# rasmusab/bayes.js

Measured on AMD Instinct MI355X. Metric: posterior draws/sec (= param-updates/sec), higher is better.
Workload: dtype f64

## Files before the change

bayes.js_amd/amwg_ctypes.py:

```python
import bisect
import ctypes as C
import os

import numpy as np

HERE = os.path.dirname(os.path.abspath(__file__))
LIB_PATH = os.environ.get("AMWG_LIB") or os.path.join(HERE, "csrc", "libamwg.so")
MODEL_ID = {"normal": 1, "beta_bern": 2, "hier_normal": 3, "pois_glm": 4}


class ParamDesc(C.Structure):
    _fields_ = [("type", C.c_int32), ("len", C.c_int32), ("top", C.c_int32), ("multidim", C.c_int32),
                ("lower", C.c_double), ("upper", C.c_double)]


class CompOpt(C.Structure):
    _fields_ = [("prop_log_scale", C.c_double), ("max_adaptation", C.c_double), ("initial_adaptation", C.c_double),
                ("target_accept_rate", C.c_double), ("batch_size", C.c_double), ("is_adapting", C.c_int32)]


class ModelDesc(C.Structure):
    _fields_ = [("model", C.c_int32), ("n_obs", C.c_int32), ("x", C.POINTER(C.c_double)), ("y", C.POINTER(C.c_double)),
                ("g", C.POINTER(C.c_int32)), ("G", C.c_int32), ("K", C.c_int32), ("hyper", C.c_double * 8)]

# ... 2 lines not shown


class Options(C.Structure):
    _fields_ = [("chains", C.c_int64), ("seed", C.c_uint64), ("chain_offset", C.c_uint64), ("device", C.c_int32),
                ("lanes_per_chain", C.c_int32), ("block_threads", C.c_int32), ("steps_per_launch", C.c_int32),
                ("exact_division", C.c_int32), ("group_local", C.c_int32), ("full_evaluation", C.c_int32), ("test_bound_shift", C.c_int32), ("sufficient_statistics", C.c_int32)]


class UserModel(C.Structure):
    _fields_ = [("source", C.c_char_p), ("n_arrays", C.c_int32), ("arrays", C.POINTER(C.POINTER(C.c_double))),
                ("array_len", C.POINTER(C.c_int64)), ("array_type", C.POINTER(C.c_int32)), ("n_derived", C.c_int32), ("lds_bytes", C.c_int32), ("lds_bytes_one_lane", C.c_int32),
                ("parallel", C.c_int32), ("max_threads", C.c_int32), ("work_per_eval", C.c_double), ("work_one_lane", C.c_double),
                ("rows_n_obs", C.c_int32), ("rows_groups", C.c_int32), ("rows_sweep", C.c_int32)]


EXPORTS = ["amwg_last_sample_dataset_histogram", "amwg_set_histogram", "amwg_histogram_info", "amwg_sample_summarize","amwg_sample_summarize_async", "amwg_summary_info", "amwg_create_user_datasets", "amwg_compile_user_datasets", "amwg_create_datasets", "amwg_create_datasets_ragged", "amwg_num_datasets", "amwg_dataset_n_obs", "amwg_last_sample_dataset_moments", "amwg_last_sample_dataset_diagnostics", "amwg_last_sample_dataset_quantiles", "amwg_kernel_name", "amwg_summation_order", "amwg_group_gather_draws", "amwg_group_comm_info", "amwg_comm_unique_id", "amwg_comm_create", "amwg_comm_info", "amwg_comm_gather_draws", "amwg_comm_moments", "amwg_comm_destroy", "amwg_code_cache_stats", "amwg_tuning", "amwg_group_moments", "amwg_group_diagnostics", "amwg_group_quantiles", "amwg_last_sample_quantiles", "amwg_fp64_peak", "amwg_set_state", "amwg_last_sample_diagnostics", "amwg_create_user", "amwg_compile_user", "amwg_num_recorded", "amwg_create", "amwg_burn", "amwg_burn_async", "amwg_sample", "amwg_sample_async", "amwg_fetch_draws", "amwg_fetch_draws_slices", "amwg_sample_device", "amwg_set_adapting", "amwg_get_state", "amwg_info", "amwg_chain_diag", "amwg_last_sample_moments", "amwg_sync", "amwg_num_components", "amwg_num_chains", "amwg_launch_info", "amwg_destroy", "amwg_last_error", "amwg_version", "amwg_exp", "amwg_log", "amwg_uniform"]
SELFTEST_EXPORTS = ["amwg_histogram_check", "amwg_summaries_check","amwg_fold_check","amwg_dataset_quantiles_check", "amwg_prefault_selftest", "amwg_math1", "amwg_math2", "amwg_hypot3", "amwg_log1p", "amwg_expm1", "amwg_two_valued_sum_check", "amwg_pow", "amwg_ld_host", "amwg_ld_device", "amwg_device_eval"]

_lib = None


def lib():
    global _lib
    if _lib is None:
        if not os.path.exists(LIB_PATH):
            raise RuntimeError("libamwg.so is missing: run `python -c 'import __graft_entry__ as g; g.build()'`")
        L = C.CDLL(LIB_PATH)
        vp, i32, i64, u64, dbl = C.c_void_p, C.c_int32, C.c_int64, C.c_uint64, C.c_double
        pd, pi32, pi64, pu64 = C.POINTER(dbl), C.POINTER(i32), C.POINTER(i64), C.POINTER(u64)
        L.amwg_create.argtypes = [C.POINTER(ModelDesc), C.POINTER(ParamDesc), i32, pd, C.POINTER(CompOpt),
                                  C.POINTER(Options), C.POINTER(vp)]
# ... 18 lines not shown
        L.amwg_last_sample_dataset_histogram.argtypes = [vp, pd, i32, pu64]
        L.amwg_set_histogram.argtypes = [vp, pd, i32]
        L.amwg_histogram_info.argtypes = [vp, pi32, C.POINTER(C.c_size_t)]
        L.amwg_set_adapting.argtypes = [vp, i32]
        L.amwg_get_state.argtypes = [vp, pd, C.c_size_t]
        L.amwg_info.argtypes = [vp, pd, pi32, pi32, pi32, pi64, pi64]
        L.amwg_chain_diag.argtypes = [vp, pu64, pd, pi32]
        L.amwg_last_sample_moments.argtypes = [vp, pd, pd]
        L.amwg_sync.argtypes = [vp]
        L.amwg_num_components.argtypes = [vp]
        L.amwg_num_chains.argtypes = [vp]
        L.amwg_num_chains.restype = i64
        L.amwg_launch_info.argtypes = [vp, pi32, pi32, pi32, pi32, pi32, pd]
        L.amwg_kernel_name.argtypes = [vp]
        L.amwg_summation_order.argtypes = [vp]
        L.amwg_kernel_name.restype = C.c_char_p
        L.amwg_destroy.argtypes = [vp]
        L.amwg_last_error.restype = C.c_char_p
        L.amwg_version.restype = C.c_char_p
        L.amwg_exp.restype = dbl
        L.amwg_exp.argtypes = [dbl]
        L.amwg_log.restype = dbl
        L.amwg_log.argtypes = [dbl]
        L.amwg_uniform.restype = dbl
        L.amwg_uniform.argtypes = [u64, u64, u64]
        L.amwg_compile_user.argtypes = [C.c_char_p, i32, i32, C.c_char_p, C.POINTER(C.c_size_t)]
        L.amwg_code_cache_stats.argtypes = [pi64, pi64, C.c_char_p, C.c_size_t]
        L.amwg_create_user.argtypes = [C.POINTER(UserModel), C.POINTER(ParamDesc), i32, pd, C.POINTER(CompOpt),
                                       C.POINTER(Options), C.POINTER(vp)]
        L.amwg_create_user_datasets.argtypes = [C.POINTER(UserModel), i32, C.POINTER(ParamDesc), i32, pd, C.POINTER(CompOpt), C.POINTER(Options), C.POINTER(vp)]
# ... 328 lines not shown
        return out

    def tuning(self):
        L = lib()
        L.amwg_tuning.argtypes = [C.c_void_p, C.POINTER(C.c_int32), C.POINTER(C.c_double), C.c_int32]
        lanes, ms = (C.c_int32 * 16)(), (C.c_double * 16)()
        n = L.amwg_tuning(self.h, lanes, ms, 16)
        return [(lanes[i], ms[i]) for i in range(min(n, 16))]

    def launch_info(self):
        v = [C.c_int32() for _ in range(5)]
        ms = C.c_double()
        _check(lib().amwg_launch_info(self.h, *[C.byref(x) for x in v], C.byref(ms)))
        return {"lanes_per_chain": v[0].value, "block_threads": v[1].value, "grid_blocks": v[2].value,
                "lds_bytes": v[3].value, "n_launches": v[4].value, "kernel_ms": ms.value, "kernel": (lib().amwg_kernel_name(self.h) or b"").decode(),
                "summation_order": lib().amwg_summation_order(self.h), "datasets": lib().amwg_num_datasets(self.h)}


def _edges_per_value(edges, PR):
    e = np.asarray(edges, dtype=np.float64)
    if e.ndim == 1:
        e = np.broadcast_to(e, (PR, e.size))
    if e.ndim != 2 or e.shape[0] != PR or e.shape[1] < 1:
        raise AmwgError("edges must be [bins + 1] or [%d recorded values][bins + 1], got shape %s" % (PR, e.shape))
    return np.ascontiguousarray(e)


def histogram_check(draws, D, edges, window_rows=0, counts=None, device=0):
    dr = np.ascontiguousarray(draws, dtype=np.float64)
    rows, PR, Cn = dr.shape
    e = _edges_per_value(edges, PR)
# ... 169 lines not shown
```

bayes.js_amd/csrc/amwg_diag.hip:

```cpp
#include <cmath>
#include <cstdarg>
#include <cstdio>

#include "amwg_build_id.h"
#include "amwg_fold.h"
#include "amwg_host.h"
#include "amwg_math.h"
#include "amwg_philox.h"

using namespace amwg;

namespace {
__global__ void chain_halves_kernel(const double *draws, int64_t rows, int PR, int64_t C, double *out) {
  const int64_t c = (int64_t)blockIdx.x * blockDim.x + threadIdx.x;
  const int p = blockIdx.y;
  if (c >= C) return;
  const int64_t half = rows / 2;
  for (int h = 0; h < 2; ++h) {
    const int64_t r0 = h * half, r1 = r0 + half;
    double m = 0, m2 = 0;
    for (int64_t r = r0; r < r1; ++r) welford_add(draws[(r * PR + p) * C + c], r - r0 + 1, m, m2);
    out[((size_t)(h * 2 + 0) * PR + p) * C + c] = m;
    out[((size_t)(h * 2 + 1) * PR + p) * C + c] = half > 1 ? m2 / (double)(half - 1) : 0.0;
  }
// ... 332 lines not shown
int amwg_num_components(const amwg_sampler *s) { return s ? s->P : 0; }
int amwg_num_recorded(const amwg_sampler *s) { return s ? s->P + s->D : 0; }
int64_t amwg_num_chains(const amwg_sampler *s) { return s ? s->C : 0; }

int amwg_launch_info(const amwg_sampler *s, int32_t *lanes, int32_t *block, int32_t *grid, int32_t *lds, int32_t *n_launches, double *kernel_ms) {
  if (!s) return amwg_fail(AMWG_EINVAL, "amwg_launch_info: null sampler");
  if (lanes) *lanes = s->plan.lanes;
  if (block) *block = s->plan.block;
  if (grid) *grid = s->plan.grid;
  if (lds) *lds = s->plan.lds;
  if (n_launches) *n_launches = s->n_launches;
  if (kernel_ms) *kernel_ms = s->kernel_ms;
  return AMWG_OK;
}

int amwg_summation_order(const amwg_sampler *s) {
  if (!s) return amwg_fail(AMWG_EINVAL, "amwg_summation_order: null sampler");
  return info(s->plan.variant).certified ? 1 : s->plan.lanes;
}

const char *amwg_kernel_name(const amwg_sampler *s) {
  if (!s) { (void)amwg_fail(AMWG_EINVAL, "amwg_kernel_name: null sampler"); return ""; }
  amwg_sampler *m = const_cast<amwg_sampler *>(s);
  if (m->kernel_name.empty()) {
    const LaunchPlan &p = s->plan;
    const int cls = p.block <= 256 ? 256 : (p.block <= 512 ? 512 : 1024);
    const std::string variant_name = std::string(info(p.variant).name) + (s->n_datasets > 1 ? "_ds" : "");
    const char *name = variant_name.c_str();
    static const char *const fam[] = {"NormalModel", "BetaBernModel", "HierNormalModel", "PoisGlmModel"};
    char buf[96];
// ... 37 lines not shown
```

bayes.js_amd/csrc/amwg_kernel.h:

```cpp
#pragma once
#if !defined(__HIPCC_RTC__)
#include <hip/hip_runtime.h>
#endif

#include "amwg_div.h"
#include "amwg_ld.h"
#include "amwg_philox.h"
#include "amwg_types.h"

namespace amwg {

struct LdsLayout {
  uint32_t data, state, pls, cnt, tot, cc, adapt, pl, idx, perm, total, stride, logpls, bc, xw;
};
__host__ __device__ inline LdsLayout lds_layout(size_t data_bytes, int P, int CPB, int max_top, int n_named, bool multi = false) {
  LdsLayout L;
  uint32_t o = 0;
  L.stride = (uint32_t)P | 1u;
  L.data = o;  o += (uint32_t)((data_bytes + 15) & ~(size_t)15);
  L.state = o; o += L.stride * CPB * 8;
  L.pls = o;   o += L.stride * CPB * 8;
  L.cnt = o;   o += L.stride * CPB * 8;
  L.tot = o;   o += (L.stride * CPB * 4 + 15) & ~15u;
  L.cc = o;    o += (uint32_t)P * sizeof(CompConst);
  L.adapt = o; o += ((uint32_t)P + 7) & ~7u;
  L.pl = o;    o += (uint32_t)n_named * 20u;
  o = (o + 15) & ~15u;
  L.idx = o;   o += (max_top > 1) ? (((uint32_t)max_top * CPB * (max_top > kByteTop ? 2u : 1u) + 15) & ~15u) : 0;
  L.perm = o;  o += (n_named > kPackedNamed) ? (((uint32_t)n_named * CPB * 2u + 15) & ~15u) : 0;
  L.logpls = o; o += multi ? L.stride * CPB * 8 : 0;
  L.bc = o;     o += multi ? ((L.stride * CPB * 4 + 15) & ~15u) : 0;
  L.xw = o;     o += multi ? 2u * 16u * 8u : 0;
  L.total = (o + 15) & ~15u;
  return L;
}

template <class Model, bool FAST, int G, int U = Model::kUnroll>
__device__ __forceinline__ double pass_over_data(const typename Model::Pass &ps, int n_obs, int sub, double acc) {
  const int n_full = n_obs / G, rem = n_obs % G;
  int k = 0;
  for (; k + U <= n_full; k += U) {
    double t[U];
#pragma unroll
    for (int u = 0; u < U; ++u) t[u] = Model::template term<FAST>(ps, (k + u) * G + sub);
#pragma unroll
    for (int u = 0; u < U; ++u) acc += t[u];
  }
// ... 228 lines not shown

__device__ inline __attribute__((noinline)) int certified_test_wide(double dA, double eta, double u) {
  const double lo = dA - eta, hi = dA + eta;
  if (hi < -746.0) return -1;
  if (lo >= 0.0) return 1;
  if (!(eta < 0x1p+9) || !(u > 0x1p-60)) return 0;
  if (exp_v8(lo) * (1.0 - 0x1p-50) > u) return 1;
  if (exp_v8(hi) * (1.0 + 0x1p-50) < u) return -1;
  return 0;
}
__device__ __forceinline__ int certified_test(double dA, double eta, double ex, double u) {
  if (eta < 0x1p-7) return (ex * (1.0 - eta) > u && (u > 0.0 || dA > -700.0)) ? 1 : (ex * (1.0 + eta) < u ? -1 : 0);
  return certified_test_wide(dA, eta, u);
}

template <class Rng>
__device__ __forceinline__ double rnorm_js(Rng &rng, double mean, double sd) {
  constexpr int GU = Rng::kLanesPerChain;
  double u, v, q;
  bool again;
  do {
    u = rng.next();
    v = 1.7156 * (rng.next() - 0.5);
    const double x = u - 0.449871;
    const double y = __builtin_fabs(v) + 0.386595;
    q = x * x + y * (0.19600 * y - 0.25472 * x);
    again = false;
    if (chain_true<GU>(q > 0.27597)) again = chain_true<GU>(q > 0.27846) || chain_true<GU>(v * v > -4 * log_v8_cold(u) * u * u);
  } while (again);
  return (v / u) * sd + mean;
}

// ... 10 lines not shown
};
__device__ __forceinline__ uint32_t perm_get(uint64_t perm, int i) { return (uint32_t)(perm >> (4 * i)) & 0xFu; }
__device__ __forceinline__ uint64_t perm_swap(uint64_t perm, int i, int j) {
  const uint64_t d = ((perm >> (4 * i)) ^ (perm >> (4 * j))) & 0xFull;
  return perm ^ (d << (4 * i)) ^ (d << (4 * j));
}

__device__ __forceinline__ double js_max2(double a, double b) {
  if (a != a || b != b) return __builtin_nan("");
  if (a == b) return (a == 0 && __builtin_signbit(a)) ? b : a;
  return a > b ? a : b;
}

template <class M, int G, bool GL, bool SW = false> struct RngOf { using type = CoopStream<G>; };
template <class M, int G> struct RngOf<M, G, true, false> { using type = typename M::Stream; };
template <class M, int G> struct RngOf<M, G, false, true> { using type = typename M::SweepStream; };
template <class M, class = void> struct DynamicLdsOf { static constexpr bool value = false; };
template <class M> struct DynamicLdsOf<M, void_of<decltype(M::kDynamicLds)>> { static constexpr bool value = M::kDynamicLds; };
template <class M, bool GL> struct DataBytesOf {
  static __device__ __forceinline__ size_t get(const DataRef &d, int lanes, int threads) {
    if constexpr (DynamicLdsOf<M>::value) return M::lds_bytes_of(d, lanes, threads);
    else return M::lds_bytes(d.n_obs, d.G, lanes);
  }
};
template <class M> struct DataBytesOf<M, true> { static __device__ __forceinline__ size_t get(const DataRef &d, int, int threads) { return M::gl_lds_bytes(d.pad, threads / 64); } };

#if defined(__HIP_DEVICE_COMPILE__)
typedef const StepArgs __attribute__((address_space(4))) *cold_args_ptr;
__device__ __forceinline__ cold_args_ptr cold_args() {
  cold_args_ptr p = (cold_args_ptr)__builtin_amdgcn_kernarg_segment_ptr();
// ... 104 lines not shown
template <class M, class = void> struct MirrorCheckOf { static constexpr bool value = false; };
template <class M> struct MirrorCheckOf<M, void_of<decltype(M::kMirrorCheck)>> { static constexpr bool value = M::kMirrorCheck; };

template <class Model, int G, int BT = 256, bool GL = false, bool SW = false, bool CT = false>
__device__ __forceinline__ void step_body(const StepArgs &a, unsigned char *smem) {
  constexpr int kPassU = SW ? (CertNeedsRows<Model>::value ? 2 : 4) : (BT >= 1024 ? 4 : 8);
  const int tid = threadIdx.x, nt = blockDim.x;
  constexpr bool kMulti = G > 64;
  if (!kMulti && a.cpb > 0 && nt != 64) { device_error(a, kErrReplicasNeedOneWave); return; }
  if (a.n_steps > 65535) { device_error(a, kErrLaunchTooLong); return; }
  const int CPB = kMulti ? G / 64 : ((a.cpb > 0 && a.cpb < nt / G) ? a.cpb : nt / G);
  const int c_raw = kMulti ? tid / 64 : tid / G;
  const int c_in = c_raw < CPB ? c_raw : CPB - 1, sub = tid % G;
  const int P = a.pl.P;
  const int n_named = a.pl.n_params;
  const LdsLayout L = lds_layout(DataBytesOf<Model, GL>::get(a.d, G, nt), P, CPB, a.pl.max_top, n_named, kMulti);

  const unsigned char *data_lds = smem + L.data;
  double *Sblk = reinterpret_cast<double *>(smem + L.state);
  CompConst *cc = reinterpret_cast<CompConst *>(smem + L.cc);
  uint8_t *adapt = smem + L.adapt;
  int32_t *pl_base = reinterpret_cast<int32_t *>(smem + L.pl), *pl_len = pl_base + n_named, *pl_top = pl_len + n_named, *pl_multidim = pl_top + n_named, *pl_inner = pl_multidim + n_named;
  const bool wide_idx = a.pl.max_top > kByteTop, wide_perm = n_named > kPackedNamed;
  const IndexColumn idx{smem + L.idx + (wide_idx ? 2 * c_in : c_in), CPB, wide_idx};
  const IndexColumn pcol{smem + L.perm + 2 * c_in, CPB, true};
  double *SDme = reinterpret_cast<double *>(smem + L.pls) + (size_t)c_in * L.stride;
  int2 *CNTme = reinterpret_cast<int2 *>(smem + L.cnt) + (size_t)c_in * L.stride;
  uint32_t *TOTme = reinterpret_cast<uint32_t *>(smem + L.tot) + (size_t)c_in * L.stride;
  double *LOGPLSme = reinterpret_cast<double *>(smem + L.logpls) + (size_t)c_in * L.stride;
  int32_t *BCme = reinterpret_cast<int32_t *>(smem + L.bc) + (size_t)c_in * L.stride;
  CrossWave xw{reinterpret_cast<double *>(smem + L.xw), 0};
// ... 11 lines not shown
  const bool counter = sub == 0 && c_raw < CPB;
  const int64_t C = a.C;

  double *Sme = Sblk + (size_t)c_in * L.stride;
  for (int p = 0; p < P; ++p) {
    Sme[p] = a.ch.state[p * C + cl];
    SDme[p] = exp_v8(a.ch.prop_log_scale[p * C + cl]);
    CNTme[p] = make_int2(a.ch.acceptance_count[p * C + cl], a.ch.iterations_since_adaption[p * C + cl]);
    TOTme[p] = 0u;
    if constexpr (kMulti) { LOGPLSme[p] = a.ch.prop_log_scale[p * C + cl]; BCme[p] = a.ch.batch_count[p * C + cl]; }
  }
  const StateView S{Sme};
  uint64_t perm = wide_perm ? 0ull : a.ch.perm[cl];
  if (wide_perm)
    for (int k = 0; k < n_named; ++k) pcol.set(k, (int)a.ch.perm16[(int64_t)k * C + cl]);
  typename RngOf<Model, G, GL, SW>::type rng;
  if constexpr (GL) rng.init(a.seed, a.chain_offset + (uint64_t)cl, a.ch.rng_n[cl], tid, reinterpret_cast<double *>(smem + L.data + Model::gl_lds_bytes(a.d.pad, 0)) + (size_t)(tid >> 6) * 256);
  else if constexpr (SW) rng.init(a.seed, a.chain_offset + (uint64_t)cl, a.ch.rng_n[cl], tid, reinterpret_cast<double *>(smem + L.data + Model::window_offset(a.d, nt / 64)) + (size_t)(tid >> 6) * 256);
  else rng.init(a.seed, a.chain_offset + (uint64_t)cl, a.ch.rng_n[cl], tid);
  double lp_curr = a.ch.lp_curr[cl];
  __syncthreads();
  constexpr bool kCert = CT && CertifiedAt<Model, G>::value && !GL && (SW == CertNeedsRows<Model>::value);
  static_assert(kCert == CT, "a certified kernel is instantiated for a model that has no certified value at this lane count");
  constexpr bool kRefOrder = kCert && G > 1 && RefOrderOf<Model>::value;
  auto expression = [&]() -> double {
    if constexpr (kRefOrder) return Model::template reference_order<G>(cache, S, a.mc, a.d, data_lds, sub);
    else if constexpr (!GL) return log_post<Model, G, kPassU>(S, a, data_lds, sub, xw, cache);
    else return 0.0;
  };
  if constexpr (!GL) { if (a.init_lp) lp_curr = expression(); }
  double lpA = lp_curr, epsA = 0.0;
  bool lp_exact = true;
  if constexpr (kCert) { if (!a.init_lp) { epsA = a.ch.lp_eps[cl]; lp_exact = epsA == 0.0; } }
// ... 595 lines not shown
        if (counter) (void)__hip_atomic_fetch_add(&TOTme[comp], 1u + ((now != old) ? 0x10000u : 0u), __ATOMIC_RELAXED, __HIP_MEMORY_SCOPE_WORKGROUP);
        if (slot + 1 < P_stepped) nx = prefetch(next_comp());
        continue;
      }
      AMWG_PHASE(14);
      const double cur = me.cur;
      const bool in_sweep = kSweep && sw_left > 0;
      double prop;
      if (in_sweep) prop = lane_value(sw_prop, comp - sb);
      else {
        prop = rnorm_js(rng, cur, me.sd);
        if (chain_true<G>(k_type == kTypeInt)) prop = js_round(prop);
      }
      const bool inb = chain_true<G>(!(prop < k_lower || prop > k_upper));
      double u_accept = 0.0;
      if (inb) { set_state(comp, prop); u_accept = in_sweep ? lane_value(sw_u, comp - sb) : rng.next(); }
      if (in_sweep) --sw_left;
      AMWG_PHASE(8);
      if (slot + 1 < P_stepped) nx = prefetch(next_comp());
      AMWG_PHASE(9);
      bool accepted = false;
      bool certified = false;
      [[maybe_unused]] double aud_E_prop = 0.0;
      if constexpr (kCert) {
        if (__ballot(inb) != 0ull) {
          wave_priority(0);
          const typename Model::Approx r = Model::template log_post_approx<G, BT>(cache, S, a.mc, a.d, data_lds, sub);
          wave_priority(kStepperPriority);
          AMWG_PHASE(10);
          if (inb) {
// ... 130 lines not shown
```

bayes.js_amd/csrc/amwg_plan.hip:

```cpp
#include <algorithm>
#include <cmath>
#include <cstdlib>

#include "amwg_host.h"
#include "amwg_kernel.h"
#include "amwg_models.h"

using namespace amwg;

const FamilyRow *family_of(int model) {
  static const FamilyRow rows[4] = {amwg_family_row<0>(), amwg_family_row<1>(), amwg_family_row<2>(), amwg_family_row<3>()};
  return model >= AMWG_MODEL_NORMAL && model <= AMWG_MODEL_POIS_GLM ? &rows[model - 1] : nullptr;
}

int gl_layout(const double *y, const int32_t *g, int N, int Gn, GlLayoutHost *out) {
  if (Gn < 1 || Gn > 64) return amwg_fail(AMWG_EINVAL, "group_local: 1 to 64 groups (a chain runs on one wavefront, a lane serves one group), got %d", Gn);
  std::vector<int> n(Gn, 0), L(Gn, 1), first(Gn, 0);
  for (int i = 0; i < N; ++i) {
    if (g[i] < 0 || g[i] >= Gn) return amwg_fail(AMWG_EINVAL, "group_local: g[%d] = %d outside 0..%d", i, g[i], Gn - 1);
    n[g[i]]++;
  }
  int total = Gn;
  for (;;) {
    int best = 0;
// ... 80 lines not shown
  return p.variant == Variant::HierSweep || p.variant == Variant::HierSweepCert || (s->user && p.pad > 0);
}

static uint32_t lds_of_size(const amwg_sampler *s, const LaunchPlan &p, int cpb, int n_obs) {
  const int G = p.lanes, bt = p.block;
  size_t data = 0;
  switch (p.variant) {
    case Variant::GroupLocal: data = HierGlModel::gl_lds_bytes(p.pad, bt / 64); break;
    case Variant::HierSweep: case Variant::HierSweepCert: data = HierNormalModel::rows_lds_bytes(p.pad, bt / 64, s->d.G); break;
    case Variant::Step: case Variant::StepCert:
      data = (s->model == AMWG_MODEL_NORMAL && G == 1) ? (p.pad ? NormalModel::one_lane_tile_bytes(n_obs) : 0) : family_of(s->model)->lds_bytes(n_obs, s->d.G, G);
      break;
    default:
      data = p.pad ? HierNormalModel::rows_lds_bytes(p.pad, bt / 64, s->user_rows_groups) : (size_t)(G == 1 ? s->user_lds_one_lane : s->user_lds);
  }
  return G > 64 ? lds_layout(data, s->P, G / 64, s->pl.max_top, s->n_params, true).total : lds_layout(data, s->P, cpb ? cpb : bt / G, s->pl.max_top, s->n_params).total;
}

static uint32_t lds_of(const amwg_sampler *s, const LaunchPlan &p, int cpb = 0) {
  if (s->n_datasets <= 1) return lds_of_size(s, p, cpb, s->d.n_obs);
  uint32_t most = 0;
  int last = -1;
  for (int n : s->ds_n_obs) {
    if (n == last) continue;
    most = std::max(most, lds_of_size(s, p, cpb, n));
    last = n;
  }
  return most;
}

static int priced_n_obs(const amwg_sampler *s) {
// ... 43 lines not shown
  return bytes / (64 * sizeof(double));
}
static int size_wave_scratch(amwg_sampler *s) {
  const char *env = getenv("AMWG_WAVE_SCRATCH");
  if ((env && env[0] == '0') || s->plan.lanes != 1) return AMWG_OK;
  const size_t lines = (size_t)s->plan.grid * (size_t)(s->plan.block / 64);
  if (s->d.wave_scratch && lines <= wave_scratch_lines(s)) return AMWG_OK;
  double *p = nullptr;
  TRYB(dev_alloc(s, &p, lines * 64));
  if (s->d.wave_scratch) {
    for (auto it = s->dev_allocs.begin(); it != s->dev_allocs.end(); ++it)
      if (*it == s->d.wave_scratch) { (void)hipFree(*it); s->dev_allocs.erase(it); break; }
  }
  s->d.wave_scratch = p;
  return AMWG_OK;
}

int choose_geometry(const amwg_sampler *s, int lanes, int n_cus, size_t max_lds, LaunchPlan *out) {
  const amwg_options &o = s->opt;
  const int max_bt = s->user ? s->user_max_threads : family_of(s->model)->max_threads;
  const int64_t cpd = chains_per_dataset(s);
  bool lds_short = false;
  auto fits = [&](int bt, int G) {
    if (bt > max_bt || bt % G != 0) return false;
    if (cpd && cpd % chains_per_workgroup(G, bt) != 0) return false;
    const LaunchPlan p = variant_for(s, G, bt, max_lds);
    if (cpd && lds_of(s, p) > max_lds) lds_short = true;
    if (lds_of(s, p) > max_lds || (bt > 512 && row_layout(s, variant_for(s, G, 512, max_lds)))) return false;
    return !(G == 1 && info(p.variant).certified && !o.block_threads && bt > (p.variant == Variant::UserStepCert ? 256 : 512));
  };
// ... 42 lines not shown
  }
  if (lanes == 0 && best.lanes > 1 && cost1 > 0 && cost1 <= 1.12 * best_cost) best = one;
  if (!best.lanes && cpd && lds_short) {
    int d_max = 0;
    for (int d = 1; d < s->n_datasets; ++d) if (s->ds_n_obs[d] > s->ds_n_obs[d_max]) d_max = d;
    return amwg_fail(AMWG_EINVAL, "no launch geometry fits dataset %d, the largest (n_obs = %d): every workgroup is given the LDS of the largest dataset, and with lanes %d (0 = any), block %d (0 = any) "
                     "that is more than %zu bytes", d_max, s->ds_n_obs[d_max], lanes, o.block_threads, max_lds);
  }
  if (!best.lanes && cpd)
    return amwg_fail(AMWG_EINVAL, "no launch geometry serves whole datasets: the chains of a workgroup (block_threads / lanes_per_chain, or 1 for a chain on several wavefronts) must divide "
                     "cpd = %lld chains per dataset; asked for lanes %d (0 = any), block %d (0 = any), %zu bytes of LDS", (long long)cpd, lanes, o.block_threads, max_lds);
  if (!best.lanes) return amwg_fail(AMWG_EINVAL, "no launch geometry fits: the model needs more than %zu bytes of LDS", max_lds);
  const int CPB = best.lanes > 64 ? 1 : (best.cpb ? best.cpb : best.block / best.lanes);
  best.grid = (int)((s->C + CPB - 1) / CPB);
  best.lds = (int)lds_of(s, best, best.cpb);
  *out = best;
  return AMWG_OK;
}

int adopt_plan(amwg_sampler *s, const LaunchPlan &p) {
  s->plan = p;
  s->d.pad = p.pad;
  if (s->user) {
    if (s->n_datasets > 1) {
      const int cpw = chains_per_workgroup(p.lanes, p.block);
      const int64_t cpd = chains_per_dataset(s);
      if (p.cpb || p.pad || (p.variant != Variant::UserStep && p.variant != Variant::UserStepCert) || cpd % cpw != 0)
        return amwg_fail(AMWG_EINVAL, "internal: a plan of %d lanes in workgroups of %d (cpb %d, pad %d) for a closure on datasets of %lld chains", p.lanes, p.block, p.cpb, p.pad, (long long)cpd);
      s->ds_blocks_per_dataset = (int)(cpd / cpw);
    }
// ... 91 lines not shown
```

bayes.js_amd/csrc/amwg_rtc.hip:

```cpp
#include <hip/hiprtc.h>
#include <fcntl.h>
#include <sys/stat.h>
#include <unistd.h>

#include <cstdio>
#include <cstdlib>
#include <cstring>
#include <map>
#include <mutex>

#include "amwg_host.h"

extern "C" {
extern const char amwg_hdr_stdint[], amwg_hdr_types[], amwg_hdr_math[], amwg_hdr_div[], amwg_hdr_ld[], amwg_hdr_philox[],
    amwg_hdr_kernel[], amwg_hdr_user[], amwg_hdr_twoval[], amwg_hdr_kval[], amwg_hdr_trig[], amwg_hdr_pass[], amwg_hdr_rows[], amwg_hdr_window[], amwg_hdr_gtail[],
    amwg_hdr_user_kernels[], amwg_hdr_user_dataset[];
}

static std::string user_program(const char *source, int lanes, int block) {
  return "#include \"amwg_kernel.h\"\n#include \"amwg_user.h\"\n#define AMWG_USER_LANES " + std::to_string(lanes) + "\n#define AMWG_USER_BLOCK " + std::to_string(block) + "\n" +
         source + "\n#include \"amwg_user_kernels.h\"\n";
}

namespace {
struct CacheKey { uint64_t h1, h2, h3; uint64_t len; };
CacheKey hash_key(const std::vector<std::string> &parts) {
  CacheKey k{0xcbf29ce484222325ull, 0x84222325cbf29ce4ull, 0x9e3779b97f4a7c15ull, 0};
  for (const std::string &p : parts) {
    for (unsigned char c : p) {
// ... 54 lines not shown
  if (!f) { close(fd); (void)remove(tmp.c_str()); return; }
  const uint64_t hdr[4] = {k.h2, k.h3, k.len, payload_sum(code)}, n = code.size();
  const bool ok = fwrite(kCacheMagic, 1, 8, f) == 8 && fwrite(hdr, 8, 4, f) == 4 && fwrite(&n, 8, 1, f) == 1 && fwrite(code.data(), 1, code.size(), f) == code.size();
  if (fclose(f) != 0 || !ok || rename(tmp.c_str(), file.c_str()) != 0) (void)remove(tmp.c_str());
}
std::atomic<int> g_cache_hits{0}, g_cache_misses{0};
}

static void dump_code_object(const std::vector<char> &code) {
  if (const char *dump = getenv("AMWG_DUMP_CODE_OBJECT")) {
    if (FILE *f = fopen(dump, "wb")) { fwrite(code.data(), 1, code.size(), f); fclose(f); }
  }
}

static int compile_user(const char *source, int lanes, int block, const char *arch, std::vector<char> *code, bool datasets, bool use_cache = true) {
  static const char *names[] = {"amwg_stdint.h", "amwg_types.h", "amwg_math.h", "amwg_div.h", "amwg_ld.h", "amwg_philox.h", "amwg_kernel.h", "amwg_user.h",
                                "amwg_twoval.h", "amwg_kval.h", "amwg_trig.h", "amwg_pass.h", "amwg_rows.h", "amwg_window.h", "amwg_gtail.h", "amwg_user_kernels.h", "amwg_user_dataset.h"};
  const char *texts[] = {amwg_hdr_stdint, amwg_hdr_types, amwg_hdr_math, amwg_hdr_div, amwg_hdr_ld, amwg_hdr_philox, amwg_hdr_kernel, amwg_hdr_user,
                         amwg_hdr_twoval, amwg_hdr_kval, amwg_hdr_trig, amwg_hdr_pass, amwg_hdr_rows, amwg_hdr_window, amwg_hdr_gtail, amwg_hdr_user_kernels, amwg_hdr_user_dataset};
  constexpr int kHeaders = (int)(sizeof(texts) / sizeof(texts[0]));
  const std::string prog_src = user_program(source, lanes, block);
#if defined(AMWG_AUDIT)
  const char *const kOpts[] = {"-O3", "-std=c++17", "-ffp-contract=off", "-fno-fast-math", "-Wno-unused-value", "-DAMWG_AUDIT=1"};
#elif defined(AMWG_X_PHASES)
  const char *const kOpts[] = {"-O3", "-std=c++17", "-ffp-contract=off", "-fno-fast-math", "-Wno-unused-value", "-DAMWG_X_PHASES=1"};
#else
  const char *const kOpts[] = {"-O3", "-std=c++17", "-ffp-contract=off", "-fno-fast-math", "-Wno-unused-value", "-falign-loops=64"};
#endif
  static const char *const kDatasetsOpt = "-DAMWG_USER_DATASETS=1";
  std::string dir = cache_dir(), file;
  CacheKey key{};
  if (!dir.empty()) {
    int rt_major = 0, rt_minor = 0;
// ... 109 lines not shown
```

bayes.js_amd/csrc/amwg_rtc_headers.c:

```c
#define AMWG_TEXT(sym, file)                                                        \
  __asm__(".section .rodata\n.global " #sym "\n.type " #sym ", @object\n" #sym ":\n" \
          ".incbin \"" file "\"\n.byte 0\n.size " #sym ", .-" #sym "\n.text\n")
AMWG_TEXT(amwg_hdr_stdint, "amwg_stdint.h");
AMWG_TEXT(amwg_hdr_types, "amwg_types.h");
AMWG_TEXT(amwg_hdr_math, "amwg_math.h");
AMWG_TEXT(amwg_hdr_div, "amwg_div.h");
AMWG_TEXT(amwg_hdr_ld, "amwg_ld.h");
AMWG_TEXT(amwg_hdr_philox, "amwg_philox.h");
AMWG_TEXT(amwg_hdr_kernel, "amwg_kernel.h");
AMWG_TEXT(amwg_hdr_user, "amwg_user.h");
AMWG_TEXT(amwg_hdr_twoval, "amwg_twoval.h");
AMWG_TEXT(amwg_hdr_kval, "amwg_kval.h");
AMWG_TEXT(amwg_hdr_trig, "amwg_trig.h");
AMWG_TEXT(amwg_hdr_pass, "amwg_pass.h");
AMWG_TEXT(amwg_hdr_rows, "amwg_rows.h");
AMWG_TEXT(amwg_hdr_window, "amwg_window.h");
AMWG_TEXT(amwg_hdr_gtail, "amwg_gtail.h");
AMWG_TEXT(amwg_hdr_user_kernels, "amwg_user_kernels.h");
AMWG_TEXT(amwg_hdr_user_dataset, "amwg_user_dataset.h");
```

bayes.js_amd/csrc/amwg_run.hip:

```cpp
#include <dlfcn.h>
#include <sys/mman.h>

#include <cmath>
#include <cstddef>
#include <cstdlib>
#include <mutex>
#include <unordered_map>

#include "../../include/amwg_selftest.h"
#include "amwg_fold.h"
#include "amwg_histogram.h"
#include "amwg_host.h"
#include "amwg_kernel.h"
#include "amwg_dataset.h"
#include "amwg_user_dataset.h"

using namespace amwg;

int use_device(int device) {
  int ndev = 0;
  hipError_t e = hipGetDeviceCount(&ndev);
  if (e != hipSuccess || ndev < 1) return amwg_fail(AMWG_EHIP, "no HIP device available (%s)", hipGetErrorString(e));
  HIP_TRY(hipSetDevice(device));
  return AMWG_OK;
// ... 32 lines not shown
  const LaunchPlan &p = s->plan;
  if (p.cpb > 0 && p.block != 64) return amwg_fail(AMWG_EINVAL, "internal: %d chains per workgroup of %d threads (replicated chains need one-wavefront workgroups)", p.cpb, p.block);
  if (p.lanes == 1 && s->d.wave_scratch && wave_scratch_lines(s) < (size_t)p.grid * (size_t)(p.block / 64))
    return amwg_fail(AMWG_EINVAL, "internal: a wave scratch of %zu lines for %d workgroups of %d threads (one line per wavefront)", wave_scratch_lines(s), p.grid, p.block);
  if (chunk > 65535) return amwg_fail(AMWG_EINVAL, "internal: launches of %lld steps (at most 65535)", (long long)chunk);
  StepArgs a{};
  a.C = s->C;
  a.seed = s->opt.seed;
  a.chain_offset = s->opt.chain_offset;
  a.thin = (int32_t)thin;
  a.draws = d_draws;
  a.cc = s->d_cc;
  a.is_adapting = s->d_adapt;
  a.pl = s->pl;
  a.cpb = p.cpb;
  a.sweep_update_by_update = s->opt.full_evaluation == 2 ? 1 : 0;
  a.certified = info(p.variant).certified ? 1 : 0;
  a.bound_scale = std::ldexp(1.0, s->opt.test_bound_shift);
  a.audit_adversarial = 0;
#if defined(AMWG_AUDIT)
  { const char *e = getenv("AMWG_AUDIT_ADVERSARIAL"); a.audit_adversarial = (e && e[0] == '1') ? 1 : 0; }
#endif
  a.mc = s->mc;
  a.d = s->d;
  if (p.lanes != 1) a.d.wave_scratch = nullptr;
  a.ch = s->ch;
  DatasetArgs ds{};
  if (s->n_datasets > 1 && !s->user) {
    if (!s->ds_kernel || s->ds_blocks_per_dataset < 1 || (int64_t)s->ds_blocks_per_dataset * s->n_datasets != p.grid)
      return amwg_fail(AMWG_EINVAL, "internal: %d workgroups for %d datasets of %d workgroups each", p.grid, s->n_datasets, s->ds_blocks_per_dataset);
// ... 387 lines not shown
```

bayes.js_amd/csrc/amwg_sampler.h:

```cpp
#pragma once
#include <hip/hip_runtime.h>

#include <cstdint>
#include <string>
#include <utility>
#include <vector>

#include "../../include/amwg.h"
#include "amwg_types.h"

typedef void (*step_kernel_t)(const amwg::StepArgs);
namespace amwg { struct DatasetArgs; struct DatasetConsts; }
typedef void (*dataset_kernel_t)(const amwg::StepArgs, const amwg::DatasetArgs);

enum class Variant : uint8_t {
  Step, StepCert, HierSweep, HierSweepCert, GroupLocal,
  UserStep, UserStepCert, UserSweep, UserSweepCert
};
struct LaunchPlan {
  int lanes = 0, block = 0, grid = 0, lds = 0, cpb = 0;
  Variant variant = Variant::Step;
  int pad = 0;
};

struct amwg_sampler {
  int device = 0;
  hipStream_t stream = nullptr;
  hipEvent_t ev0 = nullptr, ev1 = nullptr;
  int model = 0, P = 0, n_params = 0;
  int64_t C = 0;
  amwg_options opt{};
  amwg::ParamLayout pl{};
  amwg::ModelConsts mc{};
  amwg::DataRef d{};
  amwg::ChainArrays ch{};
  std::vector<void *> dev_allocs;
  amwg::CompConst *d_cc = nullptr;
// ... 45 lines not shown
```

bayes.js_amd/csrc/amwg_types.h:

```cpp
#pragma once
#include "amwg_stdint.h"

namespace amwg {

constexpr int kPackedNamed = 16;
constexpr int kByteTop = 256;
constexpr int kMaxIndex = 65535;
constexpr int kInlineUserArrays = 16;
constexpr int kTypeReal = 0, kTypeInt = 1, kTypeBinary = 2, kTypeFixed = 3;

struct StateView {
  const double *base;
#if defined(__HIPCC__)
  __host__ __device__ __forceinline__
#else
  inline
#endif
  double operator()(int p) const { return base[p]; }
};

struct CompConst {
  double lower, upper, max_adaptation, initial_adaptation, target_accept_rate;
  double batch_size;
  int32_t type;
// ... 54 lines not shown
  int64_t C;
  uint64_t seed, chain_offset;
  int32_t n_steps, thin;
  int64_t step0;
  double *draws;
  int64_t row0;
  const CompConst *cc;
  const uint8_t *is_adapting;
  int32_t init_lp;
  int32_t finalize_lp;
  int32_t certified;
  double bound_scale;
  int32_t audit_adversarial;
  int32_t sweep_update_by_update;
  int32_t cpb;
  ParamLayout pl;
  ModelConsts mc;
  DataRef d;
  ChainArrays ch;
};

}
```

include/amwg.h:

```cpp
#ifndef AMWG_H
#define AMWG_H

#include <stddef.h>
#include <stdint.h>

#ifdef __cplusplus
extern "C" {
#endif

#define AMWG_OK 0
#define AMWG_EINVAL (-1)
#define AMWG_EHIP (-2)
#define AMWG_ESIZE (-3)

enum {
  AMWG_MODEL_NORMAL = 1,
  AMWG_MODEL_BETA_BERN = 2,
  AMWG_MODEL_HIER_NORMAL = 3,
  AMWG_MODEL_POIS_GLM = 4
};

enum { AMWG_REAL = 0, AMWG_INT = 1, AMWG_BINARY = 2, AMWG_FIXED = 3 };

typedef struct {
// ... 135 lines not shown
int amwg_comm_info(amwg_comm *c, int32_t *n_ranks, int32_t *rank, int32_t *device);
int amwg_comm_gather_draws(amwg_sampler *s, amwg_comm *c, int32_t root, double *dst_device, size_t capacity_bytes, int64_t *counts);
int amwg_comm_moments(amwg_sampler *s, amwg_comm *c, double *mean, double *sd);
int amwg_comm_destroy(amwg_comm *c);

int amwg_tuning(const amwg_sampler *s, int32_t *lanes, double *ms, int32_t cap);

int amwg_sync(amwg_sampler *s);
int amwg_num_components(const amwg_sampler *s);
int amwg_num_recorded(const amwg_sampler *s);
int64_t amwg_num_chains(const amwg_sampler *s);
int amwg_launch_info(const amwg_sampler *s, int32_t *lanes_per_chain, int32_t *block_threads, int32_t *grid_blocks,
                     int32_t *lds_bytes, int32_t *n_launches, double *kernel_ms);
const char *amwg_kernel_name(const amwg_sampler *s);
int amwg_summation_order(const amwg_sampler *s);
int amwg_destroy(amwg_sampler *s);
const char *amwg_last_error(void);
const char *amwg_version(void);

double amwg_exp(double x);
double amwg_log(double x);
double amwg_uniform(uint64_t seed, uint64_t chain, uint64_t index);
int amwg_fp64_peak(int32_t device, double *lane_ops_per_s);

#ifdef __cplusplus
}
#endif
#endif
```

Measured before the change: 1.483 billion.

## Buffer Philox uniforms in an LDS ring with wave-wide refills for one-lane chains

For one-lane-per-chain stepping kernels, uniforms now come from a per-thread ring buffer in LDS. The wave refills it cooperatively, generating Philox blocks only while some lane is short, and the normal sampler's rejection loop runs wave-synchronously with predicated draws. The aim is to cut divergence from lanes calling Philox at different times and to amortize each four-word Philox block across two uniforms. In exchange it adds LDS use, ballot loops and extra bookkeeping. The ring is only granted when occupancy is not reduced, and it can be disabled with AMWG_RING=0.

```diff
diff --git a/bayes.js_amd/amwg_ctypes.py b/bayes.js_amd/amwg_ctypes.py
--- a/bayes.js_amd/amwg_ctypes.py
+++ b/bayes.js_amd/amwg_ctypes.py
@@ -40,7 +40,7 @@
                 ("rows_n_obs", C.c_int32), ("rows_groups", C.c_int32), ("rows_sweep", C.c_int32)]
 
 
-EXPORTS = ["amwg_last_sample_dataset_histogram", "amwg_set_histogram", "amwg_histogram_info", "amwg_sample_summarize","amwg_sample_summarize_async", "amwg_summary_info", "amwg_create_user_datasets", "amwg_compile_user_datasets", "amwg_create_datasets", "amwg_create_datasets_ragged", "amwg_num_datasets", "amwg_dataset_n_obs", "amwg_last_sample_dataset_moments", "amwg_last_sample_dataset_diagnostics", "amwg_last_sample_dataset_quantiles", "amwg_kernel_name", "amwg_summation_order", "amwg_group_gather_draws", "amwg_group_comm_info", "amwg_comm_unique_id", "amwg_comm_create", "amwg_comm_info", "amwg_comm_gather_draws", "amwg_comm_moments", "amwg_comm_destroy", "amwg_code_cache_stats", "amwg_tuning", "amwg_group_moments", "amwg_group_diagnostics", "amwg_group_quantiles", "amwg_last_sample_quantiles", "amwg_fp64_peak", "amwg_set_state", "amwg_last_sample_diagnostics", "amwg_create_user", "amwg_compile_user", "amwg_num_recorded", "amwg_create", "amwg_burn", "amwg_burn_async", "amwg_sample", "amwg_sample_async", "amwg_fetch_draws", "amwg_fetch_draws_slices", "amwg_sample_device", "amwg_set_adapting", "amwg_get_state", "amwg_info", "amwg_chain_diag", "amwg_last_sample_moments", "amwg_sync", "amwg_num_components", "amwg_num_chains", "amwg_launch_info", "amwg_destroy", "amwg_last_error", "amwg_version", "amwg_exp", "amwg_log", "amwg_uniform"]
+EXPORTS = ["amwg_ring_uniforms", "amwg_last_sample_dataset_histogram", "amwg_set_histogram", "amwg_histogram_info", "amwg_sample_summarize","amwg_sample_summarize_async", "amwg_summary_info", "amwg_create_user_datasets", "amwg_compile_user_datasets", "amwg_create_datasets", "amwg_create_datasets_ragged", "amwg_num_datasets", "amwg_dataset_n_obs", "amwg_last_sample_dataset_moments", "amwg_last_sample_dataset_diagnostics", "amwg_last_sample_dataset_quantiles", "amwg_kernel_name", "amwg_summation_order", "amwg_group_gather_draws", "amwg_group_comm_info", "amwg_comm_unique_id", "amwg_comm_create", "amwg_comm_info", "amwg_comm_gather_draws", "amwg_comm_moments", "amwg_comm_destroy", "amwg_code_cache_stats", "amwg_tuning", "amwg_group_moments", "amwg_group_diagnostics", "amwg_group_quantiles", "amwg_last_sample_quantiles", "amwg_fp64_peak", "amwg_set_state", "amwg_last_sample_diagnostics", "amwg_create_user", "amwg_compile_user", "amwg_num_recorded", "amwg_create", "amwg_burn", "amwg_burn_async", "amwg_sample", "amwg_sample_async", "amwg_fetch_draws", "amwg_fetch_draws_slices", "amwg_sample_device", "amwg_set_adapting", "amwg_get_state", "amwg_info", "amwg_chain_diag", "amwg_last_sample_moments", "amwg_sync", "amwg_num_components", "amwg_num_chains", "amwg_launch_info", "amwg_destroy", "amwg_last_error", "amwg_version", "amwg_exp", "amwg_log", "amwg_uniform"]
 SELFTEST_EXPORTS = ["amwg_histogram_check", "amwg_summaries_check","amwg_fold_check","amwg_dataset_quantiles_check", "amwg_prefault_selftest", "amwg_math1", "amwg_math2", "amwg_hypot3", "amwg_log1p", "amwg_expm1", "amwg_two_valued_sum_check", "amwg_pow", "amwg_ld_host", "amwg_ld_device", "amwg_device_eval"]
 
 _lib = None
@@ -89,6 +89,7 @@
         L.amwg_launch_info.argtypes = [vp, pi32, pi32, pi32, pi32, pi32, pd]
         L.amwg_kernel_name.argtypes = [vp]
         L.amwg_summation_order.argtypes = [vp]
+        L.amwg_ring_uniforms.argtypes = [vp]
         L.amwg_kernel_name.restype = C.c_char_p
         L.amwg_destroy.argtypes = [vp]
         L.amwg_last_error.restype = C.c_char_p
@@ -447,7 +448,8 @@
         _check(lib().amwg_launch_info(self.h, *[C.byref(x) for x in v], C.byref(ms)))
         return {"lanes_per_chain": v[0].value, "block_threads": v[1].value, "grid_blocks": v[2].value,
                 "lds_bytes": v[3].value, "n_launches": v[4].value, "kernel_ms": ms.value, "kernel": (lib().amwg_kernel_name(self.h) or b"").decode(),
-                "summation_order": lib().amwg_summation_order(self.h), "datasets": lib().amwg_num_datasets(self.h)}
+                "summation_order": lib().amwg_summation_order(self.h), "datasets": lib().amwg_num_datasets(self.h),
+                "ring_uniforms": lib().amwg_ring_uniforms(self.h)}
 
 
 def _edges_per_value(edges, PR):
diff --git a/bayes.js_amd/csrc/amwg_diag.hip b/bayes.js_amd/csrc/amwg_diag.hip
--- a/bayes.js_amd/csrc/amwg_diag.hip
+++ b/bayes.js_amd/csrc/amwg_diag.hip
@@ -370,6 +370,11 @@
   return AMWG_OK;
 }
 
+int amwg_ring_uniforms(const amwg_sampler *s) {
+  if (!s) return amwg_fail(AMWG_EINVAL, "amwg_ring_uniforms: null sampler");
+  return s->plan.ring;
+}
+
 int amwg_summation_order(const amwg_sampler *s) {
   if (!s) return amwg_fail(AMWG_EINVAL, "amwg_summation_order: null sampler");
   return info(s->plan.variant).certified ? 1 : s->plan.lanes;
diff --git a/bayes.js_amd/csrc/amwg_kernel.h b/bayes.js_amd/csrc/amwg_kernel.h
--- a/bayes.js_amd/csrc/amwg_kernel.h
+++ b/bayes.js_amd/csrc/amwg_kernel.h
@@ -6,14 +6,15 @@
 #include "amwg_div.h"
 #include "amwg_ld.h"
 #include "amwg_philox.h"
+#include "amwg_ring.h"
 #include "amwg_types.h"
 
 namespace amwg {
 
 struct LdsLayout {
-  uint32_t data, state, pls, cnt, tot, cc, adapt, pl, idx, perm, total, stride, logpls, bc, xw;
+  uint32_t data, state, pls, cnt, tot, cc, adapt, pl, idx, perm, total, stride, logpls, bc, xw, ring;
 };
-__host__ __device__ inline LdsLayout lds_layout(size_t data_bytes, int P, int CPB, int max_top, int n_named, bool multi = false) {
+__host__ __device__ inline LdsLayout lds_layout(size_t data_bytes, int P, int CPB, int max_top, int n_named, bool multi = false, size_t ring_bytes = 0) {
   LdsLayout L;
   uint32_t o = 0;
   L.stride = (uint32_t)P | 1u;
@@ -31,6 +32,8 @@
   L.logpls = o; o += multi ? L.stride * CPB * 8 : 0;
   L.bc = o;     o += multi ? ((L.stride * CPB * 4 + 15) & ~15u) : 0;
   L.xw = o;     o += multi ? 2u * 16u * 8u : 0;
+  o = (o + 15) & ~15u;
+  L.ring = o;   o += (uint32_t)ring_bytes;
   L.total = (o + 15) & ~15u;
   return L;
 }
@@ -289,8 +292,32 @@
   return certified_test_wide(dA, eta, u);
 }
 
+template <class R, class = void> struct WaveRefillOf { static constexpr bool value = false; };
+template <class R> struct WaveRefillOf<R, void_of<decltype(R::kWaveRefill)>> { static constexpr bool value = R::kWaveRefill; };
+
+template <class Rng>
+__device__ __forceinline__ double rnorm_wave(Rng &rng, double mean, double sd) {
+  double u = 1.0, v = 0.0;
+  bool active = true;
+  do {
+    double un, vr;
+    rng.next2_if(active, un, vr);
+    const double vn = 1.7156 * (vr - 0.5);
+    const double x = un - 0.449871;
+    const double y = __builtin_fabs(vn) + 0.386595;
+    const double q = x * x + y * (0.19600 * y - 0.25472 * x);
+    bool again = false;
+    if (active && q > 0.27597) again = q > 0.27846 || vn * vn > -4 * log_v8_cold(un) * un * un;
+    u = active ? un : u;
+    v = active ? vn : v;
+    active = again;
+  } while (__ballot(active) != 0ull);
+  return (v / u) * sd + mean;
+}
+
 template <class Rng>
 __device__ __forceinline__ double rnorm_js(Rng &rng, double mean, double sd) {
+  if constexpr (WaveRefillOf<Rng>::value) return rnorm_wave(rng, mean, sd);
   constexpr int GU = Rng::kLanesPerChain;
   double u, v, q;
   bool again;
@@ -331,6 +358,9 @@
 
 template <class M, int G, bool GL, bool SW = false> struct RngOf { using type = CoopStream<G>; };
 template <class M, int G> struct RngOf<M, G, true, false> { using type = typename M::Stream; };
+template <bool USER> struct OneLaneStream { using type = RingStream; };
+template <> struct OneLaneStream<true> { using type = CoopStream<1>; };
+template <class M> struct RngOf<M, 1, false, false> { using type = typename OneLaneStream<M::kUser>::type; };
 template <class M, int G> struct RngOf<M, G, false, true> { using type = typename M::SweepStream; };
 template <class M, class = void> struct DynamicLdsOf { static constexpr bool value = false; };
 template <class M> struct DynamicLdsOf<M, void_of<decltype(M::kDynamicLds)>> { static constexpr bool value = M::kDynamicLds; };
@@ -465,7 +495,9 @@
   const int c_in = c_raw < CPB ? c_raw : CPB - 1, sub = tid % G;
   const int P = a.pl.P;
   const int n_named = a.pl.n_params;
-  const LdsLayout L = lds_layout(DataBytesOf<Model, GL>::get(a.d, G, nt), P, CPB, a.pl.max_top, n_named, kMulti);
+  using Rng = typename RngOf<Model, G, GL, SW>::type;
+  constexpr bool kRing = WaveRefillOf<Rng>::value;
+  const LdsLayout L = lds_layout(DataBytesOf<Model, GL>::get(a.d, G, nt), P, CPB, a.pl.max_top, n_named, kMulti, kRing ? ring_bytes(a.ring_uniforms, nt) : 0);
 
   const unsigned char *data_lds = smem + L.data;
   double *Sblk = reinterpret_cast<double *>(smem + L.state);
@@ -507,9 +539,10 @@
   uint64_t perm = wide_perm ? 0ull : a.ch.perm[cl];
   if (wide_perm)
     for (int k = 0; k < n_named; ++k) pcol.set(k, (int)a.ch.perm16[(int64_t)k * C + cl]);
-  typename RngOf<Model, G, GL, SW>::type rng;
+  Rng rng;
   if constexpr (GL) rng.init(a.seed, a.chain_offset + (uint64_t)cl, a.ch.rng_n[cl], tid, reinterpret_cast<double *>(smem + L.data + Model::gl_lds_bytes(a.d.pad, 0)) + (size_t)(tid >> 6) * 256);
   else if constexpr (SW) rng.init(a.seed, a.chain_offset + (uint64_t)cl, a.ch.rng_n[cl], tid, reinterpret_cast<double *>(smem + L.data + Model::window_offset(a.d, nt / 64)) + (size_t)(tid >> 6) * 256);
+  else if constexpr (kRing) rng.init(a.seed, a.chain_offset + (uint64_t)cl, a.ch.rng_n[cl], tid, reinterpret_cast<double *>(smem + L.ring), nt, a.ring_uniforms);
   else rng.init(a.seed, a.chain_offset + (uint64_t)cl, a.ch.rng_n[cl], tid);
   double lp_curr = a.ch.lp_curr[cl];
   __syncthreads();
@@ -1135,6 +1168,10 @@
       }
       const bool inb = chain_true<G>(!(prop < k_lower || prop > k_upper));
       double u_accept = 0.0;
+      if constexpr (kRing) {
+        if (inb) set_state(comp, prop);
+        u_accept = rng.next_if(inb);
+      } else
       if (inb) { set_state(comp, prop); u_accept = in_sweep ? lane_value(sw_u, comp - sb) : rng.next(); }
       if (in_sweep) --sw_left;
       AMWG_PHASE(8);
diff --git a/bayes.js_amd/csrc/amwg_plan.hip b/bayes.js_amd/csrc/amwg_plan.hip
--- a/bayes.js_amd/csrc/amwg_plan.hip
+++ b/bayes.js_amd/csrc/amwg_plan.hip
@@ -118,7 +118,8 @@
     default:
       data = p.pad ? HierNormalModel::rows_lds_bytes(p.pad, bt / 64, s->user_rows_groups) : (size_t)(G == 1 ? s->user_lds_one_lane : s->user_lds);
   }
-  return G > 64 ? lds_layout(data, s->P, G / 64, s->pl.max_top, s->n_params, true).total : lds_layout(data, s->P, cpb ? cpb : bt / G, s->pl.max_top, s->n_params).total;
+  return G > 64 ? lds_layout(data, s->P, G / 64, s->pl.max_top, s->n_params, true).total
+                : lds_layout(data, s->P, cpb ? cpb : bt / G, s->pl.max_top, s->n_params, false, ring_bytes(p.ring, bt)).total;
 }
 
 static uint32_t lds_of(const amwg_sampler *s, const LaunchPlan &p, int cpb = 0) {
@@ -192,6 +193,28 @@
   }
   s->d.wave_scratch = p;
   return AMWG_OK;
+}
+
+static void grant_ring(const amwg_sampler *s, LaunchPlan &p, int n_cus, size_t max_lds) {
+  p.ring = 0;
+  const char *env = getenv("AMWG_RING");
+  const bool one_lane_stepper = p.lanes == 1 && (p.variant == Variant::Step || p.variant == Variant::StepCert);
+  if ((env && env[0] == '0') || !one_lane_stepper) return;
+  auto resident = [&](uint32_t lds) {
+    int64_t per_cu = 2048 / p.block;
+    if (lds > 0 && (int64_t)(max_lds / lds) < per_cu) per_cu = (int64_t)(max_lds / lds);
+    const int64_t has = ((int64_t)p.grid + n_cus - 1) / (n_cus > 0 ? n_cus : 1);
+    return per_cu < has ? per_cu : has;
+  };
+  const int64_t without = resident((uint32_t)p.lds);
+  const int sizes[2] = {kRingUniforms, 8};
+  for (int r : sizes) {
+    if (r > kRingUniforms) continue;
+    LaunchPlan q = p;
+    q.ring = r;
+    const uint32_t lds = lds_of(s, q, q.cpb);
+    if (lds <= max_lds && resident(lds) >= without) { p.ring = r; p.lds = (int)lds; return; }
+  }
 }
 
 int choose_geometry(const amwg_sampler *s, int lanes, int n_cus, size_t max_lds, LaunchPlan *out) {
@@ -264,6 +287,7 @@
   const int CPB = best.lanes > 64 ? 1 : (best.cpb ? best.cpb : best.block / best.lanes);
   best.grid = (int)((s->C + CPB - 1) / CPB);
   best.lds = (int)lds_of(s, best, best.cpb);
+  grant_ring(s, best, n_cus, max_lds);
   *out = best;
   return AMWG_OK;
 }
diff --git a/bayes.js_amd/csrc/amwg_ring.h b/bayes.js_amd/csrc/amwg_ring.h
--- /dev/null
+++ b/bayes.js_amd/csrc/amwg_ring.h
@@ -0,0 +1,99 @@
+#pragma once
+#include "amwg_philox.h"
+
+#ifndef AMWG_RING_UNIFORMS
+#define AMWG_RING_UNIFORMS 16
+#endif
+
+namespace amwg {
+
+constexpr int kRingUniforms = AMWG_RING_UNIFORMS;
+static_assert(kRingUniforms >= 4 && (kRingUniforms & (kRingUniforms - 1)) == 0, "the ring holds a power of two of uniforms, at least two blocks");
+
+AMWG_HD uint32_t ring_slot(uint32_t pos, uint32_t R) { return pos & (R - 1u); }
+AMWG_HD uint32_t ring_unread(uint32_t rd, uint32_t wr) { return wr - rd; }
+AMWG_HD bool ring_has_room(uint32_t rd, uint32_t wr, uint32_t R) { return ring_unread(rd, wr) + 2u <= R; }
+AMWG_HD bool ring_holds(uint32_t rd, uint32_t wr, uint32_t k) { return ring_unread(rd, wr) >= k; }
+AMWG_HD uint32_t ring_index(uint32_t slot, uint32_t threads, uint32_t thread) { return slot * threads + thread; }
+AMWG_HD uint64_t ring_consumed(uint64_t nb, uint32_t rd, uint32_t wr) { return 2ull * nb - (uint64_t)ring_unread(rd, wr); }
+AMWG_HD uint64_t ring_first_block(uint64_t consumed) { return consumed >> 1; }
+AMWG_HD uint32_t ring_start(uint64_t consumed) { return (uint32_t)(consumed & 1ull); }
+AMWG_HD size_t ring_bytes(int R, int threads) { return (size_t)R * (size_t)threads * sizeof(double); }
+
+#if defined(__HIPCC__) || defined(__HIPCC_RTC__)
+struct RingStream {
+  static constexpr int kLanesPerChain = 1;
+  static constexpr bool kWaveRefill = true;
+  uint32_t k0, k1, c2, c3;
+  uint64_t nb;
+  uint32_t rd, wr;
+  double *col;
+  uint32_t nt, R;
+  static __device__ __attribute__((noinline)) Philox4 block(uint64_t b, uint32_t c2, uint32_t c3, uint32_t k0, uint32_t k1) {
+    return philox4x32_10((uint32_t)b, (uint32_t)(b >> 32), c2, c3, k0, k1);
+  }
+  __device__ __forceinline__ double &at(uint32_t pos) const { return col[ring_index(ring_slot(pos, R), nt, 0u)]; }
+  __device__ __forceinline__ void init(uint64_t seed, uint64_t chain, uint64_t consumed, int thread, double *region, int threads, int uniforms) {
+    k0 = (uint32_t)seed; k1 = (uint32_t)(seed >> 32);
+    c2 = (uint32_t)chain; c3 = (uint32_t)(chain >> 32);
+    col = region + thread;
+    nt = (uint32_t)threads;
+    R = (uint32_t)uniforms;
+    nb = ring_first_block(consumed) + 1ull;
+    rd = ring_start(consumed);
+    wr = 2u;
+    if (R) {
+      const Philox4 w = block(nb - 1ull, c2, c3, k0, k1);
+      if (rd == 0u) at(0u) = u53(w.w0, w.w1);
+      at(1u) = u53(w.w2, w.w3);
+    }
+  }
+  __device__ __forceinline__ uint64_t consumed() const { return ring_consumed(nb, rd, wr); }
+  __device__ __forceinline__ void ensure(uint32_t k) {
+    while (__ballot(!ring_holds(rd, wr, k)) != 0ull) {
+      if (ring_has_room(rd, wr, R)) {
+        const Philox4 w = block(nb, c2, c3, k0, k1);
+        at(wr) = u53(w.w0, w.w1);
+        at(wr + 1u) = u53(w.w2, w.w3);
+        nb += 1ull;
+        wr += 2u;
+      }
+    }
+  }
+  __device__ __forceinline__ double direct() {
+    const Philox4 w = block(nb - 1ull, c2, c3, k0, k1);
+    const double u = rd ? u53(w.w2, w.w3) : u53(w.w0, w.w1);
+    nb += (uint64_t)rd;
+    rd ^= 1u;
+    return u;
+  }
+  __device__ __forceinline__ double next() {
+    if (!R) return direct();
+    ensure(1u);
+    const double u = at(rd);
+    ++rd;
+    return u;
+  }
+  __device__ __forceinline__ double next_if(bool take) {
+    if (!R) return take ? direct() : 0.0;
+    ensure(take ? 1u : 0u);
+    const double u = at(rd);
+    rd += take ? 1u : 0u;
+    return take ? u : 0.0;
+  }
+  __device__ __forceinline__ void next2_if(bool take, double &a, double &b) {
+    if (!R) {
+      a = 1.0; b = 0.5;
+      if (take) { a = direct(); b = direct(); }
+      return;
+    }
+    ensure(take ? 2u : 0u);
+    const double ra = at(rd), rb = at(rd + 1u);
+    rd += take ? 2u : 0u;
+    a = take ? ra : 1.0;
+    b = take ? rb : 0.5;
+  }
+};
+#endif
+
+}
diff --git a/bayes.js_amd/csrc/amwg_rtc.hip b/bayes.js_amd/csrc/amwg_rtc.hip
--- a/bayes.js_amd/csrc/amwg_rtc.hip
+++ b/bayes.js_amd/csrc/amwg_rtc.hip
@@ -12,7 +12,7 @@
 #include "amwg_host.h"
 
 extern "C" {
-extern const char amwg_hdr_stdint[], amwg_hdr_types[], amwg_hdr_math[], amwg_hdr_div[], amwg_hdr_ld[], amwg_hdr_philox[],
+extern const char amwg_hdr_stdint[], amwg_hdr_types[], amwg_hdr_math[], amwg_hdr_div[], amwg_hdr_ld[], amwg_hdr_philox[], amwg_hdr_ring[],
     amwg_hdr_kernel[], amwg_hdr_user[], amwg_hdr_twoval[], amwg_hdr_kval[], amwg_hdr_trig[], amwg_hdr_pass[], amwg_hdr_rows[], amwg_hdr_window[], amwg_hdr_gtail[],
     amwg_hdr_user_kernels[], amwg_hdr_user_dataset[];
 }
@@ -97,9 +97,9 @@
 }
 
 static int compile_user(const char *source, int lanes, int block, const char *arch, std::vector<char> *code, bool datasets, bool use_cache = true) {
-  static const char *names[] = {"amwg_stdint.h", "amwg_types.h", "amwg_math.h", "amwg_div.h", "amwg_ld.h", "amwg_philox.h", "amwg_kernel.h", "amwg_user.h",
+  static const char *names[] = {"amwg_stdint.h", "amwg_types.h", "amwg_math.h", "amwg_div.h", "amwg_ld.h", "amwg_philox.h", "amwg_ring.h", "amwg_kernel.h", "amwg_user.h",
                                 "amwg_twoval.h", "amwg_kval.h", "amwg_trig.h", "amwg_pass.h", "amwg_rows.h", "amwg_window.h", "amwg_gtail.h", "amwg_user_kernels.h", "amwg_user_dataset.h"};
-  const char *texts[] = {amwg_hdr_stdint, amwg_hdr_types, amwg_hdr_math, amwg_hdr_div, amwg_hdr_ld, amwg_hdr_philox, amwg_hdr_kernel, amwg_hdr_user,
+  const char *texts[] = {amwg_hdr_stdint, amwg_hdr_types, amwg_hdr_math, amwg_hdr_div, amwg_hdr_ld, amwg_hdr_philox, amwg_hdr_ring, amwg_hdr_kernel, amwg_hdr_user,
                          amwg_hdr_twoval, amwg_hdr_kval, amwg_hdr_trig, amwg_hdr_pass, amwg_hdr_rows, amwg_hdr_window, amwg_hdr_gtail, amwg_hdr_user_kernels, amwg_hdr_user_dataset};
   constexpr int kHeaders = (int)(sizeof(texts) / sizeof(texts[0]));
   const std::string prog_src = user_program(source, lanes, block);
diff --git a/bayes.js_amd/csrc/amwg_rtc_headers.c b/bayes.js_amd/csrc/amwg_rtc_headers.c
--- a/bayes.js_amd/csrc/amwg_rtc_headers.c
+++ b/bayes.js_amd/csrc/amwg_rtc_headers.c
@@ -7,6 +7,7 @@
 AMWG_TEXT(amwg_hdr_div, "amwg_div.h");
 AMWG_TEXT(amwg_hdr_ld, "amwg_ld.h");
 AMWG_TEXT(amwg_hdr_philox, "amwg_philox.h");
+AMWG_TEXT(amwg_hdr_ring, "amwg_ring.h");
 AMWG_TEXT(amwg_hdr_kernel, "amwg_kernel.h");
 AMWG_TEXT(amwg_hdr_user, "amwg_user.h");
 AMWG_TEXT(amwg_hdr_twoval, "amwg_twoval.h");
diff --git a/bayes.js_amd/csrc/amwg_run.hip b/bayes.js_amd/csrc/amwg_run.hip
--- a/bayes.js_amd/csrc/amwg_run.hip
+++ b/bayes.js_amd/csrc/amwg_run.hip
@@ -70,6 +70,7 @@
   a.is_adapting = s->d_adapt;
   a.pl = s->pl;
   a.cpb = p.cpb;
+  a.ring_uniforms = p.ring;
   a.sweep_update_by_update = s->opt.full_evaluation == 2 ? 1 : 0;
   a.certified = info(p.variant).certified ? 1 : 0;
   a.bound_scale = std::ldexp(1.0, s->opt.test_bound_shift);
diff --git a/bayes.js_amd/csrc/amwg_sampler.h b/bayes.js_amd/csrc/amwg_sampler.h
--- a/bayes.js_amd/csrc/amwg_sampler.h
+++ b/bayes.js_amd/csrc/amwg_sampler.h
@@ -21,6 +21,7 @@
   int lanes = 0, block = 0, grid = 0, lds = 0, cpb = 0;
   Variant variant = Variant::Step;
   int pad = 0;
+  int ring = 0;
 };
 
 struct amwg_sampler {
diff --git a/bayes.js_amd/csrc/amwg_types.h b/bayes.js_amd/csrc/amwg_types.h
--- a/bayes.js_amd/csrc/amwg_types.h
+++ b/bayes.js_amd/csrc/amwg_types.h
@@ -92,6 +92,7 @@
   int32_t audit_adversarial;
   int32_t sweep_update_by_update;
   int32_t cpb;
+  int32_t ring_uniforms;
   ParamLayout pl;
   ModelConsts mc;
   DataRef d;
diff --git a/include/amwg.h b/include/amwg.h
--- a/include/amwg.h
+++ b/include/amwg.h
@@ -173,6 +173,7 @@
                      int32_t *lds_bytes, int32_t *n_launches, double *kernel_ms);
 const char *amwg_kernel_name(const amwg_sampler *s);
 int amwg_summation_order(const amwg_sampler *s);
+int amwg_ring_uniforms(const amwg_sampler *s);
 int amwg_destroy(amwg_sampler *s);
 const char *amwg_last_error(void);
 const char *amwg_version(void);
```

Result: no change. 1.494 billion (median of 6 runs) (+0.7%).
